# pvjosue/CWFA

Measured on AMD Instinct MI355X. Metric: volumes/sec inverse-pass @512×512×96 fp32; NLL match vs ref (1/2/4/8 GPU), higher is better.
Workload: dtype f32 (storage, accumulation, wavelets, couplings); convolution products on the bf16 matrix cores from an exact three-way bf16 split of both fp32 operands, six products per fp32 product: fp32-equivalent; plain-fp32-MFMA figure: fp32_mfma; 1 GPU; 512x512x96 volume, 4-scale CWFA (CAT blocks, 64 ch) + LRNN inverse, z=0, batch 1/GPU, random-init weights (BASELINE.json configs[2]); precision=split, parallelism=replicated x1 (independent volumes per GPU, no collective)

## Files before the change

### cwfa_amd/_lib.py

```python
import ctypes as C
import os

_HERE = os.path.dirname(os.path.abspath(__file__))
LIB_PATH = os.path.join(_HERE, "libcwfa_hip.so")

CLAMP = {"NONE": 0, "ATAN": 1, "TANH": 2, "SIGMOID": 3}
ACT = {None: 0, "none": 0, "elu": 1, "prelu": 2, "gelu": 3, "relu": 4}
CHAIN_MAX = 8

c_f32p = C.c_void_p
c_i64p = C.c_void_p
c_f64p = C.c_void_p


class AffineStage(C.Structure):
    _fields_ = [("s_raw", c_f32p), ("t", c_f32p), ("s_bs", C.c_int64), ("t_bs", C.c_int64), ("clamp_kind", C.c_int),
                ("clamp", C.c_float), ("pre_scale", C.c_float), ("t_neg_div_sqrt2", C.c_int), ("perm", c_i64p),
                ("perm_axis", C.c_int), ("gin", C.c_int)]


class Chain(C.Structure):
    _fields_ = [("n_stages", C.c_int), ("stage", AffineStage * CHAIN_MAX), ("src_c", C.c_void_p), ("src_h", C.c_void_p)]


# ... 101 lines not shown
    "cwfa_conv2d_wgrad_workspace_bytes": (i64, [i, i, i, i, i, i]),
    "cwfa_conv2d_wgrad_f32": (i, [p, p, p, p, p, i, i, i, i, i, i, i64, i64, f, p]),
    "cwfa_elu_bwd_f32": (i, [p, p, p, p, i, i64, i64, i64, i64, i64, p]),
    "cwfa_conv3d_hidden_fwd_f32": (i, [p, p, p, p, i, i, i, i, i, p]),
    "cwfa_conv3d_hidden_bwd_f32": (i, [p, p, p, p, p, p, i, i, i, i, i, p]),
    "cwfa_conv3d_input_bwd_f32": (i, [p, p, p, i, i, i, i, i, p]),
    "cwfa_conv3d_wgrad_workspace_bytes": (i64, [i, i, i, i]),
    "cwfa_conv3d_wgrad_f32": (i, [p, p, p, p, p, i, i, i, i, i, i, i, f, p]),
    "cwfa_prelu_bwd_f32": (i, [p, p, p, p, p, i, i64, i64, i64, i64, p]),
    "cwfa_plane_affine_f32": (i, [p, p, p, i, p, p, i, i, i64, i64, i64, i64, p]),
    "cwfa_bn_bwd_stats_f32": (i, [p, p, p, p, i, i, i64, i64, i64, p]),
    "cwfa_bn_act_bwd_f32": (i, [p, p, p, i, p, p, p, p, p, i, i, i64, i64, i64, i64, p]),
    "cwfa_maxpool2_bwd_f32": (i, [p, p, p, p, i, i, i, i, p]),
    "cwfa_gelu_f32": (i, [p, p, p, i64, i, p]),
    "cwfa_layernorm_bwd_f32": (i, [p, p, p, p, p, p, p, p, p, i, i64, p]),
    "cwfa_attention_bwd_f32": (i, [p, p, p, p, p, p, p, p, p, i, i, i64, p]),
    "cwfa_split_workspace_bytes": (i64, [i, i, i64]),
    "cwfa_split_input_f32": (i, [p, p, i, i, i64, i64, p, p, i64, p, i64, p]),
    "cwfa_conv_split_packed_bytes": (i64, [i, i, i]),
    "cwfa_conv_split_pack_f32": (i, [p, p, i, i, i, i, p]),
    "cwfa_conv_split_f32": (i, [p, p, p, i, i, i, i, i, i, i64, C.POINTER(ConvOpts), p]),
    "cwfa_conv3x3_split_packed_bytes": (i64, [i, i]),
    "cwfa_conv3x3_split_pack_f32": (i, [p, p, i, i, p]),
    "cwfa_conv3x3_split_f32": (i, [p, p, p, i, i, i, i, i, i64, i64, C.POINTER(ConvOpts), p]),
    "cwfa_conv7x7_split_packed_bytes": (i64, [i, i]),
    "cwfa_conv7x7_split_pack_f32": (i, [p, p, i, i, p]),
    "cwfa_conv7x7_split_f32": (i, [p, p, p, i, i, i, i, i, i64, i64, C.POINTER(ConvOpts), p]),
    "cwfa_couple_rows": (i, [i, p]),
    "cwfa_conv3x3_split_couple_f32": (i, [p, p, p, i, i, i, i, i64, C.POINTER(Couple), p]),
    "cwfa_subnet_layer_split_packed_bytes": (i64, []),
    "cwfa_subnet_layer_split_pack_f32": (i, [p, p, p, p]),
    "cwfa_subnet_layer_split_f32": (i, [p, p, p, p, p, i, i, i, i64, i64, i, p]),
    "cwfa_subnet_layer_split_tape_f32": (i, [p, p, p, p, p, p, i, i, i, i64, i64, i64, p]),
    "cwfa_subnet_layer_first_packed_bytes": (i64, []),
    "cwfa_subnet_layer_first_pack_f32": (i, [p, p, p, i, p, p]),
    "cwfa_subnet_layer_first_f32": (i, [p, p, p, p, p, p, i, i, i, i, i64, i64, i64, i, p]),
    "cwfa_extract_views_f32": (i, [p, p, p, i, i, i, i, i, i, f, f, i64, p]),
    "cwfa_eval_splits": (i64, [i, i64]),
    "cwfa_volume_extrema_f32": (i, [p, p, p, p, i, i64, i64, i64, C.POINTER(EvalAffine), p]),
    "cwfa_volume_metrics_f32": (i, [p, p, p, p, i, i64, i64, i64, C.POINTER(EvalAffine), f, f, f, p]),
    "cwfa_mip3_f32": (i, [p, p, p, p, p, p, i, i, i, i, i64, i64, i, C.POINTER(EvalAffine), C.POINTER(EvalPost), p]),
    "cwfa_projection_compose_f32": (i, [p, p, p, p, p, i, i, i, i, i, i, i, p]),
    "cwfa_roi_means_f32": (i, [p, p, p, i, i, i, i, i, i64, p]),
    "cwfa_select_positive_f32": (i, [p, i, i64, i64, i64, p, p, p, p]),
    "cwfa_prep_volumes_f16": (i, [p, p, p, i, i, i, i, i, i, i, i, i, f, f, i, p]),
    "cwfa_prep_frames_f32": (i, [p, p, i, i, i, i, i, i, i, p]),
    "cwfa_histogram_f32": (i, [p, i64, f, f, p, i, p, i, p]),
    "cwfa_prep_apply_f32": (i, [p, i64, i, f, f, i, p]),
    "cwfa_moments_f64": (i, [p, i64, d, p, p, i, p]),
    "cwfa_stack_mean_std_f32": (i, [p, p, p, i, i64, i64, p]),
    "cwfa_lion_step_f32": (i, [C.POINTER(LionTable), f, f, f, f, p, p, p]),
    "cwfa_wmse_workspace_bytes": (i64, [i64]),
    "cwfa_wmse_loss_f32": (i, [p, p, p, f, f, p, p, p, i64, p]),
    "cwfa_select_nonzero_f32": (i, [p, i, i64, i64, i64, p, p, p, p]),
    "cwfa_deconv_spectrum_mul_c64": (i, [p, p, p, i, i64, i, i, p]),
    "cwfa_deconv_project_f32": (i, [p, p, i, i, i, i, i, i, i, i, i, i, i, p]),
    "cwfa_deconv_ratio_f32": (i, [p, p, p, p, i64, p]),
    "cwfa_deconv_clamp_f32": (i, [p, i64, p, p, f, p]),
    "cwfa_deconv_update_f32": (i, [p, p, i, i, i, i, p]),
}
del i, i64, f, d, p

_lib = None


class CwfaHipError(RuntimeError):
# ... 27 lines not shown
```

### cwfa_amd/build.py

```python
import os
import subprocess
import sys
from concurrent.futures import ThreadPoolExecutor

HERE = os.path.dirname(os.path.abspath(__file__))
CSRC = os.path.join(HERE, "csrc")
INCLUDE = os.path.join(os.path.dirname(HERE), "include")
LIB = os.path.join(HERE, "libcwfa_hip.so")
SOURCES = ["elementwise.hip", "conv2d.hip", "conv_wino.hip", "conv_wino2d.hip", "conv_split_layer.hip", "conv_split3x3.hip", "conv3d.hip", "conv3d_split.hip", "lrnn_ops.hip", "conv_bwd.hip", "eval_ops.hip", "prep_ops.hip", "optim_ops.hip", "loss_ops.hip", "deconv_ops.hip"]
HIPCC = os.environ.get("HIPCC", "/opt/rocm/bin/hipcc")
FLAGS = ["--offload-arch=gfx950", "-O3", "-fPIC", "-std=c++17", "-ffp-contract=off", "-I", INCLUDE, "-I", CSRC,
         "-Wall", "-Wno-unused-function"]


EXTRA = {"conv3d_split.hip": ["-fno-slp-vectorize"]}


def _newer(src, dst):
    return not os.path.exists(dst) or os.path.getmtime(src) > os.path.getmtime(dst)


def build_all(force=False, verbose=False):
    deps = [os.path.join(CSRC, "common.h"), os.path.join(CSRC, "conv_internal.h"), os.path.join(INCLUDE, "cwfa_hip.h"),
            os.path.abspath(__file__)]
    objs, jobs = [], []
    for s in SOURCES:
        src, obj = os.path.join(CSRC, s), os.path.join(CSRC, s.replace(".hip", ".o"))
        objs.append(obj)
        if force or _newer(src, obj) or any(_newer(d, obj) for d in deps):
            jobs.append([HIPCC, *FLAGS, *EXTRA.get(s, []), "-c", src, "-o", obj])

    def run(cmd):
        if verbose:
            print(" ".join(cmd), flush=True)
        r = subprocess.run(cmd, capture_output=True, text=True)
        if r.returncode != 0:
            raise RuntimeError(f"hipcc failed: {' '.join(cmd)}\n{r.stdout}\n{r.stderr}")
        return r.stderr

    with ThreadPoolExecutor(max_workers=4) as ex:
        for warn in ex.map(run, jobs):
            if verbose and warn.strip():
                print(warn, file=sys.stderr)
    if jobs or force or not os.path.exists(LIB) or any(_newer(o, LIB) for o in objs):
        run([HIPCC, "--offload-arch=gfx950", "-shared", "-fPIC", "-o", LIB, *objs])
    return LIB


if __name__ == "__main__":
    print(build_all(force="--force" in sys.argv, verbose=True))
```

### cwfa_amd/networks.py

```python
import glob
import math
import re

import torch
import torch.nn as nn

from . import autograd as AG
from . import ops
from .FrEIA import framework as Ff
from .FrEIA import modules as Fm
from .INN_utils import HaarTransform1D, PermuteDim
from .unet import UNet, _Packed
from .amp import amp_entry

__all__ = ["conditional_wavelet_flow", "wavelet_flow_subnetwork", "wavelet_flow_subnetwork2D",
           "wavelet_flow_subnetwork2D_first", "cond_network", "ResidualBlock", "GlobalAttention", "drop_path", "ConvNeXt",
           "LRNN", "Encoder", "subnet_initialization", "subnet_initialization_small", "zero_initialization",
           "subnet_initialization_positive", "reset_ActNorm", "reset_perm", "serialize_INN_step", "load_INN_steps",
           "HaarTransform1D", "PermuteDim", "UNet"]

networks_n_chans = 64

_CONVS = (nn.Conv2d, nn.Conv3d, nn.Linear)

# ... 81 lines not shown
        if couple is None and AG.tracking(u, conv_in, conv_out, self.block2, self.block4, self.block6):
            a = AG.subnet(self, AG.concat(list(u)) if isinstance(u, (list, tuple)) else u, conv_in, conv_out)
            if out is not None:
                raise NotImplementedError("wavelet_flow_subnetwork: `out=` views are an inference-path feature")
            return a
        P = self._packed.get
        fused = self.n_ch == 64 and all(blk[0].bias is not None and blk[2].bias is not None
                                        for blk in (self.block2, self.block4, self.block6))
        H_, W_ = (u[0] if isinstance(u, (list, tuple)) else u).shape[2:4]
        split_layers = fused and ops._split_bf16 >= 2 and 64 * H_ * W_ * 4 < 2 ** 31
        two = isinstance(u, (list, tuple))
        u1 = None
        if (two and split_layers and ops.FIRST_LAYER_COMPOSED and ops.FIRST_LAYER_FUSED_X and conv_in.kernel_size == (1, 1)
                and conv_in.in_channels <= 31 and sum(t.shape[1] for t in u) == conv_in.in_channels):
            u1 = ops.concat_channels(list(u[:-1]) + [ops.with_ones(u[-1])])
            u, two = u1[:, :-1], False
        if two and not (len(u) == 2 and ops.VIRTUAL_CAT and conv_in.kernel_size == (1, 1) and conv_in.out_channels <= 64):
            u, two = ops.concat_channels(list(u)), False
        pc_in = self._cat_bank(conv_in, u[0].shape[1]) if two else P(conv_in)
        blocked = bool(split_layers and ops.BLOCKED_MAPS and not pc_in.split and pc_in.ks == 1 and pc_in.cout == 64)
        first_form = (split_layers and ops.FIRST_LAYER_COMPOSED and not two and conv_in.kernel_size == (1, 1) and conv_in.in_channels <= 31
                      and not pc_in.split)
        fused_x = first_form and ops.FIRST_LAYER_FUSED_X
        pre = ops.first_map_of(self)
        if fused_x:
            b = None
        elif pre is not None and pre[0] is u and pre[1] is conv_in and blocked:
            b = pre[2]
        elif two:
            b = ops.conv2d(u[0], pc_in, bias=conv_in.bias, out_blocked=blocked, cat=u[1])
        else:
            b = ops.conv2d(u, pc_in, bias=conv_in.bias, out_blocked=blocked)
        pc_out = None if couple is not None else P(conv_out)
        last_reads_blocked = split_layers and ops.BLOCKED_MAPS and (couple is not None or (pc_out.split and pc_out.ks == 3))
        for i, blk in enumerate((self.block2, self.block4, self.block6)):
            if fused:
                if split_layers and i == 0 and first_form:
                    out_blocked = bool(ops.BLOCKED_MAPS)
                    b = ops.subnet_layer_first(u1 if u1 is not None else ops.with_ones(u), b, self._first3(conv_in, blk[0], blk[2]), blk[0].bias, blk[2].bias,
                                               layout=(0 if fused_x else int(blocked)) | (int(out_blocked) << 1))
                    blocked = out_blocked
                    continue
                if split_layers:
                    out_blocked = ops.BLOCKED_MAPS and (i < 2 or last_reads_blocked)
                    b = ops.subnet_layer(b, self._split3(blk[0], blk[2]), blk[0].bias, None, blk[2].bias,
                                         layout=int(blocked) | (int(out_blocked) << 1))
                    blocked = out_blocked
                else:
                    b = ops.subnet_layer(b, P(blk[0]), blk[0].bias, self._panel(blk[2]), blk[2].bias)
                continue
            h = ops.conv2d(b, P(blk[0]), bias=blk[0].bias, act="elu")
            b = ops.conv2d(h, P(blk[2]), bias=blk[2].bias, residual=b, act2="elu")
        if couple is not None:
            return ops.conv3x3_couple(b, self._couple_bank(conv_out), *couple, in_blocked=blocked)
        return ops.conv2d(b, pc_out, bias=conv_out.bias, out=out, in_blocked=blocked)

    def _cat_bank(self, conv, c1):
        w = conv.weight
        pc = self._panels.get(("cat", id(conv), c1))
        if pc is None or pc.version != w._version or pc.src_ptr != w.data_ptr() or pc.epoch != ops.pack_epoch():
            pc = self._panels[("cat", id(conv), c1)] = ops.pack_conv_weight_cat(w, c1)
        return pc

    def _couple_bank(self, conv):
        w, bias = conv.weight, conv.bias
        hit = self._panels.get(("c", id(conv)))
        if hit is not None:
# ... 459 lines not shown
```

### cwfa_amd/ops.py

```python
import ctypes as C

import torch

from . import _lib
from ._lib import AffineStage, Chain, ConvOpts, check

__all__ = ["haar1d", "haar2d", "gather", "affine", "channel_affine", "chain_inv", "chain_inv_var", "chain_inv_roi_cov", "chain_inv_samples", "rand_uniform", "rand_trunc_normal", "chain_nll_map", "nll_compose", "chain_fwd", "pack_conv_weight",
           "conv2d", "conv2d_wgrad", "elu_bwd", "set_precision", "gelu_add", "gelu_bwd", "layernorm_bwd", "attention_bwd", "plane_affine", "bn_bwd_stats", "bn_act_bwd", "maxpool2_bwd", "chain_bwd", "chain_inv_bwd", "prelu_bwd", "conv3d_1k1_backward", "pack_1x1_panel", "pack_split_layer_weight", "subnet_layer", "conv3d_1k1", "channel_stats", "bn_fold", "bn_running_update", "maxpool", "sample_stats", "layernorm_apply",
           "convnext_tail", "conv_writes_sample_stats", "attention_combine", "scale_channels", "axpby", "stage", "lion_step", "global_extrema", "wmse_loss"]


def _stream():
    return C.c_void_p(torch.cuda.current_stream().cuda_stream)


def _p(t):
    return None if t is None else C.c_void_p(t.data_ptr())


def _dev(t, name="tensor"):
    if not torch.is_tensor(t):
        raise TypeError(f"{name}: expected a torch.Tensor, got {type(t)}")
    if not t.is_cuda:
        raise RuntimeError(f"{name}: cwfa_amd runs on MI355X only -- got a {t.device} tensor (no CPU fallback exists)")
# ... 458 lines not shown
    loss = torch.zeros(1, dtype=torch.float64, device=xhat.device)
    if want_low_grad and loss_kind != 0:
        raise ValueError("chain_inv_bwd: dL/dlow is formed from an upstream gradient (loss_kind 0)")
    gz = torch.empty((B, Cc, H, W), dtype=torch.float32, device=xhat.device) if want_latent_grad else None
    glow = torch.empty((B, Cc, H, W), dtype=torch.float32, device=xhat.device) if want_low_grad else None
    check(L.cwfa_chain_inv_bwd_f32(_p(xhat), _p(gt), C.byref(ch), C.byref(gr), B, Cc, H, W, xbs, gbs, float(gscale), int(loss_kind),
                                   int(bool(accumulate)), _p(loss), _p(gz), _p(glow), _stream()), "chain_inv_bwd")
    if want_latent_grad or want_low_grad:
        return loss, gz, glow
    return loss


def chain_bwd(z, stages, grads, final_perm=None, gscale=0.0, ldscale=0.0, gz=None, want_input_grad=False, accumulate=False, gld=None):
    L = _lib.lib()
    z, zbs = planes(z, "z")
    B, Cc, H, W = z.shape
    ch, keep = _chain(stages)
    gr = _chain_grads(grads, (B, Cc, H, W))
    gzbs = 0
    if gz is not None:
        gz, gzbs = planes(gz, "gz")
    gv0 = torch.empty((B, Cc, H, W), dtype=torch.float32, device=z.device) if want_input_grad else None
    if gld is not None:
        gld = _dev(gld, "gld").contiguous()
        if gld.numel() != B:
            raise ValueError("chain_bwd: gld must hold one value per sample")
    check(L.cwfa_chain_bwd_f32(_p(z), _p(gz), C.byref(ch), C.byref(gr), _p(_idx(final_perm)), _p(gv0), B, Cc, H, W, zbs, gzbs,
                               Cc * H * W, float(gscale), float(ldscale), int(bool(accumulate)), _p(gld), _stream()), "chain_bwd")
    return gv0


class PackedConv:
    __slots__ = ("packed", "cout", "cin", "ks", "transposed", "version", "src_ptr", "split", "epoch", "version1", "src_ptr1", "cat_c1",
                 "cat_from", "short")

    def __init__(self, packed, cout, cin, ks, transposed, version, src_ptr, split=False):
        self.packed, self.cout, self.cin, self.ks = packed, cout, cin, ks
        self.transposed, self.version, self.src_ptr = transposed, version, src_ptr
        self.split = split
        self.epoch = _pack_epoch


def pack_conv_weight(w, transposed=False, direct=False):
    L = _lib.lib()
    w = _dev(w, "weight").detach().contiguous()
    if transposed:
        cin, co, kh, kw = w.shape
        if (kh, kw) != (2, 2):
            raise ValueError("only 2x2 stride-2 transposed convolutions are supported")
        cout, ks = 4 * co, 1
    else:
        cout, cin, ks, kw = w.shape
        if ks != kw:
            raise ValueError("square kernels only")
    if direct:
        pass
    elif _split_bf16 and ks == 1 and cout >= 128:
        packed = torch.empty(L.cwfa_conv_split_packed_bytes(cout, cin, ks), dtype=torch.uint8, device=w.device)
        check(L.cwfa_conv_split_pack_f32(_p(w), _p(packed), cout, cin, ks, int(transposed), _stream()), "conv_split_pack")
        return PackedConv(packed, cout, cin, ks, transposed, w._version, w.data_ptr(), split=True)
    narrow_max = 32 if single_product() else SPLIT_3X3_NARROW_MAX
    if not direct and _split_bf16 >= 2 and ks == 3 and cout >= SPLIT_3X3_MIN_COUT and (cout > 32 or (cout <= narrow_max and cin >= 29)):
        packed = torch.empty(L.cwfa_conv3x3_split_packed_bytes(cout, cin), dtype=torch.uint8, device=w.device)
        check(L.cwfa_conv3x3_split_pack_f32(_p(w), _p(packed), cout, cin, _stream()), "conv3x3_split_pack")
        return PackedConv(packed, cout, cin, ks, transposed, w._version, w.data_ptr(), split=True)
    if not direct and SPLIT_7X7 and _split_bf16 >= 2 and ks == 7 and cout <= 64 and cin >= 32:
        packed = torch.empty(L.cwfa_conv7x7_split_packed_bytes(cout, cin), dtype=torch.uint8, device=w.device)
        check(L.cwfa_conv7x7_split_pack_f32(_p(w), _p(packed), cout, cin, _stream()), "conv7x7_split_pack")
        return PackedConv(packed, cout, cin, ks, transposed, w._version, w.data_ptr(), split=True)
    n = L.cwfa_conv2d_packed_floats(cout, cin, ks)
    if n <= 0:
        raise ValueError(f"unsupported filter bank {tuple(w.shape)}")
    packed = torch.empty(n, dtype=torch.float32, device=w.device)
    check(L.cwfa_conv2d_pack_f32(_p(w), _p(packed), cout, cin, ks, int(transposed), _stream()), "conv2d_pack")
    return PackedConv(packed, cout, cin, ks, transposed, w._version, w.data_ptr())


def pack_conv_weight_cat(w, c1):
    w = _dev(w, "weight").detach()
    cout, cin, ks, kw = w.shape
    if ks != 1 or kw != 1 or cout > 64 or not (0 < c1 < cin):
        raise ValueError(f"pack_conv_weight_cat: a 1x1 bank with <= 64 outputs and 0 < c1 < Cin is needed, got {tuple(w.shape)}, c1 = {c1}")
    start = (c1 + 15) // 16 * 16
    wz = torch.zeros((cout, start + cin - c1, 1, 1), dtype=torch.float32, device=w.device)
    wz[:, :c1] = w[:, :c1]
    wz[:, start:] = w[:, c1:]
    pc = pack_conv_weight(wz)
    pc.version, pc.src_ptr = w._version, w.data_ptr()
    pc.cat_c1, pc.cat_from = c1, start
    return pc


def conv_writes_stats(pc, act=None, residual=None, act2=None, out_blocked=False, in_add=False):
    return bool(pc.split and pc.ks == 3 and act in (None, "prelu") and residual is None and act2 is None and not out_blocked
                and not (in_add and act is None))


def conv_writes_sample_stats(pc):
    return bool(pc.split and pc.ks == 7 and pc.cin <= 8)


def conv2d(x, pc, bias=None, act=None, prelu_alpha=None, residual=None, act2=None, in_scale=None, in_shift=None,
           in_add=None, out=None, in_blocked=False, out_blocked=False, cat=None, out_stats=None, out_sample_stats=None):
    L = _lib.lib()
    x, xbs = planes(x, "x")
    B, Cin, H, W = x.shape
    o = ConvOpts()
    keep = [x]
    if cat is not None:
        cat, cbs = planes(cat, "cat")
        c1 = getattr(pc, "cat_c1", None)
        if c1 is None or Cin != c1 or tuple(cat.shape) != (B, pc.cin - pc.cat_from, H, W) or in_scale is not None or in_add is not None:
            raise ValueError("conv2d: `cat` needs a bank from pack_conv_weight_cat for exactly these two inputs, and no load-side prologue")
        o.in_cat, o.in_cat_bs, o.in_cat_from, o.in_cat_c1 = cat.data_ptr(), cbs, pc.cat_from, c1
        keep.append(cat)
        Cin = pc.cin
    if Cin != pc.cin:
        raise ValueError(f"conv2d: input has {Cin} channels, filter bank expects {pc.cin}")
    up = bool(pc.transposed)
    oshape = (B, pc.cout // 4, 2 * H, 2 * W) if up else (B, pc.cout, H, W)
    if out is None:
        out = torch.empty(oshape, dtype=torch.float32, device=x.device)
        ybs = oshape[1] * oshape[2] * oshape[3]
    else:
        if tuple(out.shape) != oshape:
            raise ValueError(f"conv2d: out has shape {tuple(out.shape)}, expected {oshape}")
        out_c, ybs = planes(out, "out")
        if out_c.data_ptr() != out.data_ptr():
            raise ValueError("conv2d: `out` must have contiguous planes")
    if bias is not None:
        o.bias = _dev(bias, "bias").data_ptr()
    o.act, o.act2 = _lib.ACT[act], _lib.ACT[act2]
    if prelu_alpha is not None:
        prelu_alpha = _dev(prelu_alpha, "prelu_alpha")
        o.prelu_alpha = prelu_alpha.data_ptr()
        if prelu_alpha.numel() != 1:
            if prelu_alpha.numel() != pc.cout or not prelu_alpha.is_contiguous() or not (pc.split and pc.ks == 3):
                raise ValueError("conv2d: per-channel PReLU slopes need [Cout] contiguous values and the split-bf16 3x3 kernel")
            o.prelu_per_channel = 1
    elif "prelu" in (act, act2):
        raise ValueError("conv2d: PReLU needs prelu_alpha")
    if residual is not None:
        residual, rbs = planes(residual, "residual")
        if tuple(residual.shape) != oshape:
            raise ValueError(f"conv2d: residual {tuple(residual.shape)} != output {oshape}")
        o.residual, o.res_bs = residual.data_ptr(), rbs
        keep.append(residual)
    if in_scale is not None:
        o.in_scale, o.in_shift = _dev(in_scale).data_ptr(), _dev(in_shift).data_ptr()
        if in_scale.numel() not in (Cin, B * Cin) or in_shift.numel() != in_scale.numel():
            raise ValueError("conv2d: in_scale / in_shift must be [Cin] or [B,Cin]")
        o.in_affine_bs = Cin if (in_scale.numel() == B * Cin and B > 1) else 0
    if in_add is not None:
        in_add, abs_ = planes(in_add, "in_add")
        if tuple(in_add.shape) != tuple(x.shape):
            raise ValueError("conv2d: in_add shape mismatch")
        o.in_add, o.in_add_bs = in_add.data_ptr(), abs_
        keep.append(in_add)
    o.upshuffle2 = int(up)
    if in_blocked:
        if not (pc.split and pc.ks == 3):
            raise ValueError("conv2d: channel-blocked input is read by the split-bf16 3x3 kernel only")
        o.in_blocked8 = 1
    if out_blocked:
        ok3 = (pc.split and pc.ks == 3 and pc.cout % 8 == 0 and residual is None and act2 is None and act in (None, "prelu")
               and not split3x3_narrow(pc.cout) and not (in_add is not None and act is None))
        ok1 = not pc.split and pc.ks == 1 and pc.cout >= 33 and pc.cout % 8 == 0 and not up
        if not (ok3 or ok1):
            raise ValueError("conv2d: channel-blocked output is written by the split-bf16 3x3 kernel (bias / PReLU) and by the "
                             "direct 1x1 kernel with 40..64 output channels only")
        o.out_blocked8 = 1
    if out_stats is not None:
        if not conv_writes_stats(pc, act, residual, act2, out_blocked, in_add is not None):
            raise ValueError("conv2d: out_stats needs the split-bf16 3x3 kernel with an NCHW output and a bias / PReLU epilogue")
        if out_stats.dtype != torch.float64 or out_stats.numel() != 2 * pc.cout or not out_stats.is_cuda:
            raise ValueError("conv2d: out_stats must be a float64 [2*Cout] tensor on the HIP device")
        o.out_stats = out_stats.data_ptr()
    if out_sample_stats is not None:
        if not conv_writes_sample_stats(pc):
            raise ValueError("conv2d: out_sample_stats needs the few-channel split 7x7 kernel (a composed ConvNeXt bank with <= 8 inputs)")
        if out_sample_stats.dtype != torch.float64 or out_sample_stats.numel() != 2 * B or not out_sample_stats.is_cuda:
            raise ValueError("conv2d: out_sample_stats must be a float64 [2*B] tensor on the HIP device")
        o.out_sample_stats = out_sample_stats.data_ptr()
    rec = conv_event_sink
    if rec is not None:
        key = (pc.ks, Cin, pc.cout, H, W, B, "%s|%s|%s|%s|%s" % ("pro" if (in_scale is not None or in_add is not None) else "",
                                                                 act or "", "res" if residual is not None else "", act2 or "",
                                                                 ("up" if up else "") + ("+split" if pc.split else "")),
               in_add is not None)
        if rec.want(key):
            e0, e1 = torch.cuda.Event(enable_timing=True), torch.cuda.Event(enable_timing=True)
            e0.record()
    if pc.split and pc.ks == 7:
        if act or act2 or residual is not None or in_scale is not None or in_add is not None:
            raise ValueError("conv2d: the split-bf16 7x7 kernel has a bias-only epilogue and no load-side prologue")
        check(L.cwfa_conv7x7_split_f32(_p(x), _p(pc.packed), _p(out), B, Cin, H, W, pc.cout, xbs, ybs, C.byref(o), _stream()),
              "conv7x7_split")
    elif pc.split and pc.ks == 3:
        if split3x3_narrow(pc.cout) and (in_scale is not None or in_add is not None):
            if (H * W) % 4 == 0:
                x = plane_affine(x, in_scale, in_shift, add=in_add)
            else:
                if in_scale is not None:
                    if in_scale.numel() == Cin:
                        x = channel_affine(x, in_scale.reshape(-1), in_shift.reshape(-1))
                    else:
                        x = torch.cat([channel_affine(x[i:i + 1], in_scale.reshape(B, Cin)[i].contiguous(), in_shift.reshape(B, Cin)[i].contiguous())
                                       for i in range(B)], 0)
                if in_add is not None:
                    x = axpby(x.contiguous(), 1.0, in_add, 1.0)
            x, xbs = planes(x, "x")
            o.in_scale = o.in_shift = o.in_add = None
        check(L.cwfa_conv3x3_split_f32(_p(x), _p(pc.packed), _p(out), B, Cin, H, W, pc.cout, xbs, ybs, C.byref(o),
                                       _stream()), "conv3x3_split")
    elif pc.split:
        ws = torch.empty(L.cwfa_split_workspace_bytes(B, Cin, H * W), dtype=torch.uint8, device=x.device)
        per_sample = in_scale is not None and in_scale.numel() == B * Cin and B > 1
        check(L.cwfa_split_input_f32(_p(x), _p(ws), B, Cin, H * W, xbs, _p(in_scale), _p(in_shift), Cin if per_sample else 0,
                                     _p(in_add), in_add.stride(0) if in_add is not None else 0, _stream()), "split_input")
        o.in_scale = o.in_shift = o.in_add = None
        check(L.cwfa_conv_split_f32(_p(ws), _p(pc.packed), _p(out), B, Cin, H, W, pc.cout, pc.ks, ybs, C.byref(o), _stream()),
              "conv_split")
    else:
        check(L.cwfa_conv2d_f32(_p(x), _p(pc.packed), _p(out), B, Cin, H, W, pc.cout, pc.ks, xbs, ybs, C.byref(o),
                                _stream()), "conv2d")
    if rec is not None and rec.want(key):
# ... 44 lines not shown
    if logdet is not None:
        cp.logdet = logdet.data_ptr()
    cp.in_blocked8 = int(bool(in_blocked))
    rec = conv_event_sink
    if rec is not None:
        key = (3, Cin, pc.cout, H, W, B, "||||couple+split", False)
        if rec.want(key):
            e0, e1 = torch.cuda.Event(enable_timing=True), torch.cuda.Event(enable_timing=True)
            e0.record()
    check(L.cwfa_conv3x3_split_couple_f32(_p(u), _p(pc.packed), _p(br), B, Cin, H, W, ubs, C.byref(cp), _stream()),
          "conv3x3_split_couple")
    if rec is not None and rec.want(key):
        e1.record()
        rec.add(key, e0, e1)
    return out


BLOCKED_MAPS = True
SPLIT_7X7 = True
VIRTUAL_CAT = True
COUPLE_EPILOGUE = True


def couple_fused():
    return COUPLE_EPILOGUE and _split_bf16 >= 2


def split3x3_narrow(cout):
    return cout <= 48 or 64 < cout <= 96


SPLIT_3X3_MIN_COUT = 1
SPLIT_3X3_NARROW_MAX = 16
conv_event_sink = None


def pack_1x1_panel(w):
    L = _lib.lib()
    w = _dev(w, "weight").detach().contiguous()
    if tuple(w.shape) != (64, 64, 1, 1):
        raise ValueError("pack_1x1_panel: the fused layer kernel is specialised for 64 channels")
    panel = torch.empty(4096, dtype=torch.float32, device=w.device)
    check(L.cwfa_subnet_pack1x1_f32(_p(w), _p(panel), _stream()), "subnet_pack1x1")
    return PackedConv(panel, 64, 64, 1, False, w._version, w.data_ptr())


def pack_split_layer_weight(w3, w1):
    L = _lib.lib()
    w3 = _dev(w3, "weight").detach().contiguous()
    w1 = _dev(w1, "weight").detach().contiguous()
    if tuple(w3.shape) != (64, 64, 3, 3) or tuple(w1.shape) != (64, 64, 1, 1):
        raise ValueError("pack_split_layer_weight: 64x64x3x3 and 64x64x1x1 only")
    packed = torch.empty(L.cwfa_subnet_layer_split_packed_bytes(), dtype=torch.uint8, device=w3.device)
    check(L.cwfa_subnet_layer_split_pack_f32(_p(w3), _p(w1), _p(packed), _stream()), "subnet_layer_split_pack")
    pc = PackedConv(packed, 64, 64, 3, False, w3._version, w3.data_ptr(), split=True)
    pc.version1, pc.src_ptr1 = w1._version, w1.data_ptr()
    return pc


FIRST_LAYER_COMPOSED = True
FIRST_LAYER_FUSED_X = True


def pack_first_layer_weight(w0, b0, w3, w1, short=None):
    L = _lib.lib()
    w0, w3, w1 = _dev(w0, "w0").detach(), _dev(w3, "w3").detach(), _dev(w1, "w1").detach().contiguous()
# ... 1069 lines not shown
```

### include/cwfa_hip.h

```cpp
#ifndef CWFA_HIP_H
#define CWFA_HIP_H

#include <stdint.h>

#ifdef __cplusplus
extern "C" {
#endif

#define CWFA_VERSION 100

enum {
    CWFA_OK = 0,
    CWFA_E_INVAL = -1,
    CWFA_E_SHAPE = -2,
    CWFA_E_ALIGN = -3,
    CWFA_E_HIP = -4
};

enum { CWFA_CLAMP_NONE = 0, CWFA_CLAMP_ATAN = 1, CWFA_CLAMP_TANH = 2, CWFA_CLAMP_SIGMOID = 3 };

enum { CWFA_ACT_NONE = 0, CWFA_ACT_ELU = 1, CWFA_ACT_PRELU = 2, CWFA_ACT_GELU = 3, CWFA_ACT_RELU = 4 };

int cwfa_version(void);
const char* cwfa_last_error(void);
// ... 162 lines not shown
                           int64_t x_bs, int64_t y_bs, const cwfa_conv_opts* opts, void* stream);
int cwfa_conv_split_f32(const void* ws, const void* w_packed, float* y, int B, int Cin, int H, int W, int Cout, int ks, int64_t y_bs,
                           const cwfa_conv_opts* opts, void* stream);
int64_t cwfa_conv7x7_split_packed_bytes(int Cout, int Cin);
int cwfa_conv7x7_split_pack_f32(const float* w, void* packed, int Cout, int Cin, void* stream);
int cwfa_conv7x7_split_f32(const float* x, const void* w_packed, float* y, int B, int Cin, int H, int W, int Cout,
                           int64_t x_bs, int64_t y_bs, const cwfa_conv_opts* opts, void* stream);

typedef struct {
    const float* x;
    float* y;
    int64_t x_bs, y_bs;
    int n;
    int clamp_kind;
    float clamp, pre_scale;
    int rev;
    double* logdet;
    int in_blocked8;
} cwfa_couple;
int cwfa_couple_rows(int n, int* rows);
int cwfa_conv3x3_split_couple_f32(const float* x, const void* w_packed, const float* bias_rows, int B, int Cin, int H, int W,
                                  int64_t x_bs, const cwfa_couple* cp, void* stream);

int64_t cwfa_subnet_layer_split_packed_bytes(void);
int cwfa_subnet_layer_split_pack_f32(const float* w3, const float* w1, void* packed, void* stream);
int cwfa_subnet_layer_split_f32(const float* x, const void* packed, const float* b3, const float* b1, float* y, int B, int H,
                                int W, int64_t x_bs, int64_t y_bs, int layout, void* stream);
int64_t cwfa_subnet_layer_first_packed_bytes(void);
int cwfa_subnet_layer_first_pack_f32(const float* w3c, const float* w1, const float* w0c, int short_form, void* packed, void* stream);
int cwfa_subnet_layer_first_f32(const float* u, const float* x, const void* packed, const float* b3, const float* b1, float* y, int B,
                                int u_ch, int H, int W, int64_t u_bs, int64_t x_bs, int64_t y_bs, int layout, void* stream);
int cwfa_subnet_layer_split_tape_f32(const float* x, const void* packed, const float* b3, const float* b1, float* y, float* hid, int B,
                                     int H, int W, int64_t x_bs, int64_t y_bs, int64_t hid_bs, void* stream);

int cwfa_extract_views_f32(const float* image, const int* coords_yx, float* views, int B, int Hs, int Ws, int nviews, int sh,
                           int sw, float mean, float stdv, int64_t image_bs, void* stream);


typedef struct {
    float* ds[CWFA_CHAIN_MAX];
    float* dt[CWFA_CHAIN_MAX];
    int64_t ds_bs[CWFA_CHAIN_MAX], dt_bs[CWFA_CHAIN_MAX];
} cwfa_chain_grads;

int cwfa_chain_bwd_f32(const float* z, const float* gz, const cwfa_chain* ch, const cwfa_chain_grads* grads,
                       const int64_t* final_perm, float* gv0, int B, int C, int H, int W, int64_t z_bs, int64_t gz_bs,
                       int64_t gv0_bs, float gscale, float ldscale, int accumulate, const float* gld, void* stream);

int cwfa_chain_inv_bwd_f32(const float* xhat, const float* gt, const cwfa_chain* ch, const cwfa_chain_grads* grads, int B, int C,
                           int H, int W, int64_t xhat_bs, int64_t gt_bs, float gscale, int loss_kind, int accumulate,
                           double* loss_sum, float* gz_out, float* glow_out, void* stream);

int cwfa_affine_bwd_f32(const float* x, const float* g, const cwfa_affine_stage* st, int rev, int B, int C, int H, int W,
                        int64_t x_bs, int64_t g_bs, const float* gld, float* gx, float* gs_raw, float* gt_raw, void* stream);

int64_t cwfa_conv2d_wgrad_workspace_bytes(int B, int Cin, int H, int W, int Cout, int ks);
int cwfa_conv2d_wgrad_f32(const float* x, const float* dy, float* dw, float* db, void* workspace, int B, int Cin, int H, int W,
                          int Cout, int ks, int64_t x_bs, int64_t dy_bs, float beta, void* stream);

int cwfa_elu_bwd_f32(const float* g, const float* a, const float* add, float* y, int B, int64_t n, int64_t g_bs, int64_t a_bs,
                     int64_t add_bs, int64_t y_bs, void* stream);

int cwfa_conv3d_hidden_fwd_f32(const float* x, const float* w1, const float* b1, float* q, int B, int D, int H, int W, int K,
                               void* stream);
int cwfa_conv3d_hidden_bwd_f32(const float* dy, const float* w2, const float* q, const float* alpha, float* m, double* dalpha,
                               int B, int D, int H, int W, int K, void* stream);
// ... 98 lines not shown
```

Before: 55.50 volumes/s.

## Add persistent split-bf16 3x3 kernel for narrow subnet output convolutions

Adds a dedicated persistent kernel for the 64-to-at-most-48-channel 3x3 output convolution of the subnetworks. It stages input tiles and weight slices through LDS with double-buffered async loads overlapped with the six-product split MFMA, and walks tiles across CUs (optionally XCD-aware). It can read the channel-blocked input layout, so the preceding layers keep producing blocked maps. The trade-off is a second packed weight copy per eligible conv, and a path that only applies when the epilogue is bias-only.

Result: faster. 56.62 volumes/s (median of 6 runs) (+2.0%).

```diff
diff --git a/cwfa_amd/_lib.py b/cwfa_amd/_lib.py
--- a/cwfa_amd/_lib.py
+++ b/cwfa_amd/_lib.py
@@ -157,6 +157,9 @@
     "cwfa_subnet_layer_split_pack_f32": (i, [p, p, p, p]),
     "cwfa_subnet_layer_split_f32": (i, [p, p, p, p, p, i, i, i, i64, i64, i, p]),
     "cwfa_subnet_layer_split_tape_f32": (i, [p, p, p, p, p, p, i, i, i, i64, i64, i64, p]),
+    "cwfa_conv3x3_out_split_packed_bytes": (i64, [i]),
+    "cwfa_conv3x3_out_split_pack_f32": (i, [p, p, i, p]),
+    "cwfa_conv3x3_out_split_f32": (i, [p, p, p, p, i, i, i, i, i64, i64, i, p]),
     "cwfa_subnet_layer_first_packed_bytes": (i64, []),
     "cwfa_subnet_layer_first_pack_f32": (i, [p, p, p, i, p, p]),
     "cwfa_subnet_layer_first_f32": (i, [p, p, p, p, p, p, i, i, i, i, i64, i64, i64, i, p]),
diff --git a/cwfa_amd/build.py b/cwfa_amd/build.py
--- a/cwfa_amd/build.py
+++ b/cwfa_amd/build.py
@@ -7,7 +7,7 @@
 CSRC = os.path.join(HERE, "csrc")
 INCLUDE = os.path.join(os.path.dirname(HERE), "include")
 LIB = os.path.join(HERE, "libcwfa_hip.so")
-SOURCES = ["elementwise.hip", "conv2d.hip", "conv_wino.hip", "conv_wino2d.hip", "conv_split_layer.hip", "conv_split3x3.hip", "conv3d.hip", "conv3d_split.hip", "lrnn_ops.hip", "conv_bwd.hip", "eval_ops.hip", "prep_ops.hip", "optim_ops.hip", "loss_ops.hip", "deconv_ops.hip"]
+SOURCES = ["elementwise.hip", "conv2d.hip", "conv_wino.hip", "conv_wino2d.hip", "conv_split_layer.hip", "conv_split_out.hip", "conv_split3x3.hip", "conv3d.hip", "conv3d_split.hip", "lrnn_ops.hip", "conv_bwd.hip", "eval_ops.hip", "prep_ops.hip", "optim_ops.hip", "loss_ops.hip", "deconv_ops.hip"]
 HIPCC = os.environ.get("HIPCC", "/opt/rocm/bin/hipcc")
 FLAGS = ["--offload-arch=gfx950", "-O3", "-fPIC", "-std=c++17", "-ffp-contract=off", "-I", INCLUDE, "-I", CSRC,
          "-Wall", "-Wno-unused-function"]
@@ -21,7 +21,7 @@
 
 
 def build_all(force=False, verbose=False):
-    deps = [os.path.join(CSRC, "common.h"), os.path.join(CSRC, "conv_internal.h"), os.path.join(INCLUDE, "cwfa_hip.h"),
+    deps = [os.path.join(CSRC, "common.h"), os.path.join(CSRC, "conv_internal.h"), os.path.join(CSRC, "conv_split_out_geom.h"), os.path.join(INCLUDE, "cwfa_hip.h"),
             os.path.abspath(__file__)]
     objs, jobs = [], []
     for s in SOURCES:
diff --git a/cwfa_amd/csrc/conv_split_out.hip b/cwfa_amd/csrc/conv_split_out.hip
--- /dev/null
+++ b/cwfa_amd/csrc/conv_split_out.hip
@@ -0,0 +1,359 @@
+#include "conv_internal.h"
+#include "conv_split_out_geom.h"
+
+extern int g_cwfa_split_xcd_map;
+
+namespace {
+
+using namespace cwfa_out;
+
+constexpr int XR = TR + 2, XC = TC + 2;
+constexpr int KHB = 9984;
+constexpr int XPB = 2 * KHB;
+constexpr int XB = 3 * XPB;
+constexpr int OFF_W = 2 * XB;
+constexpr int NE = 2 * XR * XC;
+constexpr int lds_bytes(int mt) { return OFF_W + 4 * slice_bytes(mt) + 64 * mt; }
+static_assert(lds_bytes(MAX_MT) <= 160 * 1024, "LDS budget");
+
+struct OParams {
+    const float* x;
+    float* y;
+    const void* wp;
+    const float* bias;
+    int B, H, W, Cout, tiles_x, tiles_y, ntiles;
+    int64_t x_bs, y_bs;
+    int xcd_map;
+};
+
+__host__ __device__ constexpr int unit_off(int u) {
+    const int chunk = u / 9, tap = u % 9;
+    return (chunk & 1) * XB + ((tap / 3) * XC + tap % 3) * 16;
+}
+
+template <bool SIX, bool F16, bool INB, int MT>
+__global__ __launch_bounds__(512, 1) void split_out_kernel(OParams p) {
+    static_assert(MT >= 1 && MT <= MAX_MT, "one to three m-tiles");
+    constexpr int WSL = slice_bytes(MT), OFF_BIAS = OFF_W + 4 * WSL;
+    constexpr int NQ = SIX ? 3 : 1;
+    constexpr int NKB = NQ * MT;
+    constexpr int NST = 16 * MT;
+    extern __shared__ __attribute__((aligned(16))) char lds[];
+    const int tid = threadIdx.x, lane = tid & 63, wave = tid >> 6, c16 = lane & 15, g = lane >> 4;
+    const int HW = p.H * p.W;
+    const int plane = HW * 4;
+    constexpr unsigned OOB = 0x80000000u;
+
+    int epk[3], edst[3];
+    bool fin[3];
+#pragma unroll
+    for (int k = 0; k < 3; ++k) {
+        const int e = tid + k * 512;
+        fin[k] = e < NE;
+        const int c_ = e % XC, r_ = (e / XC) % XR, h_ = (e / (XR * XC)) & 1;
+        epk[k] = c_ | (r_ << 8) | (h_ << 16);
+        edst[k] = h_ * KHB + (r_ * XC + c_) * 16;
+    }
+    const bool stage2 = wave < 4;
+    auto entry_offsets = [&](bool valid, int row0, int col0, unsigned (&fo)[3]) {
+#pragma unroll
+        for (int k = 0; k < 3; ++k) {
+            const int gr = row0 + ((epk[k] >> 8) & 255) - 1, gc = col0 + (epk[k] & 255) - 1, eh = epk[k] >> 16;
+            const bool ok = valid && fin[k] && gr >= 0 && gr < p.H && gc >= 0 && gc < p.W;
+            fo[k] = !ok ? OOB : INB ? (unsigned)((eh * HW + gr * p.W + gc) * 32) : (unsigned)((eh * 8 * HW + gr * p.W + gc) * 4);
+        }
+    };
+    const bool xmap = xcd_walk(p.xcd_map, p.ntiles, (int)gridDim.x);
+    auto coords = [&](int it, int& b, int& row0, int& col0) { tile_coords(it, xmap, p.ntiles, p.tiles_x, p.tiles_y, b, row0, col0); };
+    auto load_entry = [&](f32x4 (&xv)[2], const float* base, unsigned fo, int chunk) {
+        const auto rs = CWFA_RSRC(base, 64 * plane);
+        if constexpr (INB) {
+            xv[0] = __builtin_bit_cast(f32x4, __builtin_amdgcn_raw_buffer_load_b128(rs, fo, chunk * 16 * plane, 0));
+            xv[1] = __builtin_bit_cast(f32x4, __builtin_amdgcn_raw_buffer_load_b128(rs, fo, chunk * 16 * plane + 16, 0));
+            return;
+        }
+#pragma unroll
+        for (int j = 0; j < 8; ++j)
+            xv[j >> 2][j & 3] = __builtin_bit_cast(float, __builtin_amdgcn_raw_buffer_load_b32(rs, fo, (chunk * 16 + j) * plane, 0));
+    };
+    auto store_entry = [&](auto kc, const f32x4 (&xv)[2], int buf) {
+        constexpr int k = decltype(kc)::value;
+        if (k == 2 && !stage2) return;
+        bf16x8 pc[3];
+#pragma unroll
+        for (int j = 0; j < 8; ++j) {
+            __bf16 a1, a2 = (__bf16)0.f, a3 = (__bf16)0.f;
+            cwfa_split3<SIX, F16>(xv[j >> 2][j & 3], a1, a2, a3);
+            pc[0][j] = a1; pc[1][j] = a2; pc[2][j] = a3;
+        }
+        if (fin[k]) {
+            char* dst = lds + buf * XB + edst[k];
+#pragma unroll
+            for (int q = 0; q < NQ; ++q) *reinterpret_cast<bf16x8*>(dst + q * XPB) = pc[q];
+        }
+    };
+
+    const auto rw = CWFA_RSRC(p.wp, NSL * WSL);
+    int tw = 0;
+    auto slot_off = [&](int s) { return (s & 3) * WSL + ((s & 2) ? -tw : tw); };
+    auto dma_w = [&](int s) {
+        const int so = slot_off(s), src = (s % NSL) * WSL;
+        if (wave < NKB)
+            __builtin_amdgcn_raw_ptr_buffer_load_lds(rw, (lds_ptr)(lds + OFF_W + so + wave * 1024), 16, (unsigned)tid * 16u, src, 0, 0);
+        if constexpr (NKB > 8) {
+            if (wave == 0)
+                __builtin_amdgcn_raw_ptr_buffer_load_lds(rw, (lds_ptr)(lds + OFF_W + so + 8192), 16, 8192u + (unsigned)tid * 16u, src, 0, 0);
+        }
+    };
+
+    const int alane = OFF_W + (g * 16 * MT + c16) * 16;
+    const int blane = (g & 1) * KHB + ((2 * wave) * XC + c16) * 16;
+    const bool sel = (g >> 1) != 0;
+    const f32x4* bias4 = reinterpret_cast<const f32x4*>(lds + OFF_BIAS);
+
+    f32x4 acc[MT][4];
+    bf16x8 A[2][3], Bq[4][3];
+    f32x4 xa[3][2], xb[3][2];
+    unsigned fo_c[3], fo_n[3];
+
+    auto read_a = [&](int set, int s, int mt) {
+        const int ab = alane + slot_off(s);
+#pragma unroll
+        for (int q = 0; q < NQ; ++q) A[set][q] = *reinterpret_cast<const bf16x8*>(lds + ab + (q * 64 * MT + mt * 16) * 16);
+    };
+    auto read_b = [&](int nt, int bbase) {
+#pragma unroll
+        for (int q = 0; q < NQ; ++q)
+            Bq[nt][q] = *reinterpret_cast<const bf16x8*>(lds + bbase + q * XPB + ((nt >> 1) * XC + 16 * (nt & 1)) * 16);
+    };
+    auto mfma6 = [&](f32x4& c, const bf16x8 (&a)[3], const bf16x8 (&b)[3]) {
+        if constexpr (SIX) {
+            CWFA_MFMA(a[2], b[0], c);
+            CWFA_MFMA(a[1], b[1], c);
+            CWFA_MFMA(a[0], b[2], c);
+            CWFA_MFMA(a[1], b[0], c);
+            CWFA_MFMA(a[0], b[1], c);
+        }
+        CWFA_MFMA_OP(F16, a[0], b[0], c);
+    };
+    auto bbase_of = [&](int offA, int offB) { return blane + (sel ? offB : offA); };
+
+    if (tid < 16 * MT) reinterpret_cast<float*>(lds + OFF_BIAS)[tid] = (p.bias != nullptr && tid < p.Cout) ? p.bias[tid] : 0.f;
+    int tile = blockIdx.x;
+    int tb, row0, col0;
+    coords(tile, tb, row0, col0);
+    const float* xs_cur = p.x + (int64_t)tb * p.x_bs;
+    entry_offsets(true, row0, col0, fo_c);
+    cwfa_static_for<3>([&](auto kc) { load_entry(xa[decltype(kc)::value], xs_cur, fo_c[decltype(kc)::value], 0); });
+    cwfa_static_for<3>([&](auto kc) { load_entry(xb[decltype(kc)::value], xs_cur, fo_c[decltype(kc)::value], 1); });
+    dma_w(0);
+    dma_w(1);
+    dma_w(2);
+    dma_w(3);
+    cwfa_static_for<3>([&](auto kc) { store_entry(kc, xa[decltype(kc)::value], 0); });
+    asm volatile("s_waitcnt vmcnt(0)\n\ts_waitcnt lgkmcnt(0)" ::: "memory");
+    __builtin_amdgcn_s_barrier();
+    read_a(0, 0, 0);
+    {
+        const int bb = bbase_of(unit_off(0), unit_off(1));
+#pragma unroll
+        for (int nt = 0; nt < 4; ++nt) read_b(nt, bb);
+    }
+
+    for (; tile < p.ntiles; tile += gridDim.x) {
+        const int ntile = tile + gridDim.x;
+        const bool has_next = ntile < p.ntiles;
+        int nb, nrow0, ncol0;
+        coords(has_next ? ntile : tile, nb, nrow0, ncol0);
+        const float* xs_next = p.x + (int64_t)nb * p.x_bs;
+        entry_offsets(has_next, nrow0, ncol0, fo_n);
+
+#pragma unroll
+        for (int mt = 0; mt < MT; ++mt) {
+            const f32x4 bv = bias4[mt * 4 + g];
+#pragma unroll
+            for (int nt = 0; nt < 4; ++nt) acc[mt][nt] = bv;
+        }
+
+        cwfa_static_for<NSL>([&](auto sc) {
+            constexpr int S = decltype(sc)::value, P = S % 9, PER = S / 9;
+            constexpr bool LASTP = PER == 1;
+            constexpr auto loads_in = [](int s) { return ((s % 9 >= 2 && s % 9 <= 4) || s % 9 >= 6) ? (INB ? 2 : 8) : 0; };
+            constexpr int NL = loads_in(S), NLP = loads_in((S + NSL - 1) % NSL);
+            auto issue_memory = [&]() {
+                if constexpr (S != 0) dma_w(S + 3);
+                if constexpr (P >= 2 && P <= 4) {
+                    constexpr int k = P - 2;
+                    if constexpr (!LASTP) load_entry(xa[k], xs_cur, fo_c[k], 2 * PER + 2);
+                    else load_entry(xa[k], xs_next, fo_n[k], 0);
+                }
+                if constexpr (P >= 6) {
+                    constexpr int k = P - 6;
+                    if constexpr (!LASTP) load_entry(xb[k], xs_cur, fo_c[k], 2 * PER + 3);
+                    else load_entry(xb[k], xs_next, fo_n[k], 1);
+                }
+            };
+            constexpr int NS = (S + 1) % NSL;
+            const int bbn = bbase_of(unit_off(2 * NS), unit_off(2 * NS + 1));
+            CWFA_FENCE();
+#pragma unroll
+            for (int mt = 0; mt < MT; ++mt) {
+                const int set = (S * MT + mt) & 1;
+                if (mt < MT - 1) read_a(set ^ 1, S, mt + 1);
+                else read_a(set ^ 1, S + 1, 0);
+                CWFA_FENCE();
+#pragma unroll
+                for (int np = 0; np < 4; np += 2) {
+                    mfma6(acc[mt][np], A[set], Bq[np]);
+                    mfma6(acc[mt][np + 1], A[set], Bq[np + 1]);
+                    CWFA_FENCE();
+                    if (mt == MT - 1) {
+                        read_b(np, bbn);
+                        read_b(np + 1, bbn);
+                        CWFA_FENCE();
+                    }
+                }
+                if (mt == 0) {
+                    issue_memory();
+                    CWFA_FENCE();
+                    if constexpr (P <= 2) store_entry(cwfa_ic<P>{}, xb[P], 1);
+                    if constexpr (P >= 5 && P <= 7) store_entry(cwfa_ic<P - 5>{}, xa[P - 5], 0);
+                    CWFA_FENCE();
+                }
+            }
+            asm volatile("s_waitcnt vmcnt(%0)" ::"n"(S == 0 ? NLP + NST : S == 1 ? NST : NLP + NL) : "memory");
+            asm volatile("s_waitcnt lgkmcnt(0)" ::: "memory");
+            __builtin_amdgcn_s_barrier();
+        });
+
+        dma_w(NSL + 3);
+        {
+            const auto ry = CWFA_RSRC(p.y + (int64_t)tb * p.y_bs, p.Cout * plane);
+#pragma unroll
+            for (int nt = 0; nt < 4; ++nt) {
+                const int row = row0 + 2 * wave + (nt >> 1), col = col0 + 16 * (nt & 1) + c16;
+                const bool ok = col < p.W && row < p.H;
+                const unsigned oo = (unsigned)(row * p.W + col) * 4u + (unsigned)g * 4u * (unsigned)plane;
+#pragma unroll
+                for (int mt = 0; mt < MT; ++mt)
+#pragma unroll
+                    for (int r = 0; r < 4; ++r) {
+                        const float v = acc[mt][nt][r];
+                        __builtin_amdgcn_raw_buffer_store_b32(__builtin_bit_cast(unsigned, v), ry,
+                                                              (ok && mt * 16 + 4 * g + r < p.Cout) ? oo : OOB, (mt * 16 + r) * plane, 0);
+                    }
+            }
+        }
+        tb = nb; row0 = nrow0; col0 = ncol0;
+        xs_cur = xs_next;
+        tw = 2 * WSL - tw;
+#pragma unroll
+        for (int k = 0; k < 3; ++k) fo_c[k] = fo_n[k];
+    }
+    asm volatile("s_waitcnt vmcnt(0)" ::: "memory");
+}
+
+template <bool F16>
+__global__ __launch_bounds__(256) void split_out_pack_kernel(const float* __restrict__ w, uint4* __restrict__ out, int Cout, int mt) {
+    const int i = blockIdx.x * blockDim.x + threadIdx.x;
+    const int rows = 16 * mt;
+    if (i >= NSL * 4 * rows) return;
+    const int co = i % rows, g = (i / rows) % 4, sl = i / (4 * rows);
+    unsigned short pc[3][8];
+#pragma unroll
+    for (int j = 0; j < 8; ++j) {
+        const float v = co < Cout ? w[pack_src(sl, g, j, co)] : 0.f;
+        __bf16 a1, a2, a3;
+        if constexpr (F16) {
+            cwfa_split3<false, true>(v, a1, a2, a3);
+            a2 = a3 = __builtin_bit_cast(__bf16, (unsigned short)0);
+        } else {
+            cwfa_split3<true>(v, a1, a2, a3);
+        }
+        pc[0][j] = __builtin_bit_cast(unsigned short, a1);
+        pc[1][j] = __builtin_bit_cast(unsigned short, a2);
+        pc[2][j] = __builtin_bit_cast(unsigned short, a3);
+    }
+#pragma unroll
+    for (int q = 0; q < 3; ++q) {
+        uint4 u;
+        u.x = pc[q][0] | ((unsigned)pc[q][1] << 16);
+        u.y = pc[q][2] | ((unsigned)pc[q][3] << 16);
+        u.z = pc[q][4] | ((unsigned)pc[q][5] << 16);
+        u.w = pc[q][6] | ((unsigned)pc[q][7] << 16);
+        out[pack_dst(sl, q, g, co, mt)] = u;
+    }
+}
+
+int g_out_cus = 0;
+
+template <bool SIX, bool F16, bool INB, int MT>
+int out_launch(const OParams& p, int grid, hipStream_t st) {
+    constexpr auto kern = &split_out_kernel<SIX, F16, INB, MT>;
+    const int rc = cwfa_max_lds<kern>(lds_bytes(MT), "cwfa_conv3x3_out_split_f32");
+    if (rc) return rc;
+    hipLaunchKernelGGL(kern, dim3(grid), dim3(512), lds_bytes(MT), st, p);
+    CWFA_LAUNCH_CHECK("cwfa_conv3x3_out_split_f32");
+    return CWFA_OK;
+}
+
+}
+
+extern "C" int64_t cwfa_conv3x3_out_split_packed_bytes(int Cout) {
+    if (Cout < 1 || Cout > MAX_COUT) return -1;
+    return packed_bytes(Cout);
+}
+
+extern "C" int cwfa_conv3x3_out_split_pack_f32(const float* w, void* packed, int Cout, void* stream) {
+    CWFA_REQUIRE(w && packed, CWFA_E_INVAL, "cwfa_conv3x3_out_split_pack_f32: null pointer");
+    CWFA_REQUIRE(Cout >= 1 && Cout <= MAX_COUT, CWFA_E_SHAPE, "cwfa_conv3x3_out_split_pack_f32: 1 <= Cout <= 48 (got %d)", Cout);
+    CWFA_REQUIRE(cwfa_aligned16(packed), CWFA_E_ALIGN, "cwfa_conv3x3_out_split_pack_f32: packed image must be 16-byte aligned");
+    const int mt = mt_of(Cout);
+    const dim3 grid((unsigned)((NSL * 4 * 16 * mt + 255) / 256));
+    uint4* out = reinterpret_cast<uint4*>(packed);
+    cwfa_with_operand([&](auto, auto f16) -> int {
+        hipLaunchKernelGGL(split_out_pack_kernel<f16>, grid, dim3(256), 0, (hipStream_t)stream, w, out, Cout, mt);
+        return CWFA_OK;
+    });
+    CWFA_LAUNCH_CHECK("cwfa_conv3x3_out_split_pack_f32");
+    return CWFA_OK;
+}
+
+extern "C" int cwfa_conv3x3_out_split_f32(const float* x, const void* packed, const float* bias, float* y, int B, int H, int W, int Cout,
+                                          int64_t x_bs, int64_t y_bs, int in_blocked, void* stream) {
+    CWFA_REQUIRE(Cout >= 1 && Cout <= MAX_COUT, CWFA_E_SHAPE, "cwfa_conv3x3_out_split_f32: 1 <= Cout <= 48 (got %d)", Cout);
+    CWFA_REQUIRE(B >= 0 && H >= 0 && W >= 0, CWFA_E_INVAL, "cwfa_conv3x3_out_split_f32: bad size");
+    if (B == 0 || H == 0 || W == 0) return CWFA_OK;
+    CWFA_REQUIRE(x && packed && y, CWFA_E_INVAL, "cwfa_conv3x3_out_split_f32: null pointer");
+    CWFA_REQUIRE((const void*)x != (const void*)y, CWFA_E_INVAL, "cwfa_conv3x3_out_split_f32: in-place not supported (3x3 halo)");
+    CWFA_REQUIRE(cwfa_aligned16(packed), CWFA_E_ALIGN, "cwfa_conv3x3_out_split_f32: packed image must be 16-byte aligned");
+    CWFA_REQUIRE(!in_blocked || cwfa_aligned16(x), CWFA_E_ALIGN, "cwfa_conv3x3_out_split_f32: blocked input must be 16-byte aligned");
+    CWFA_REQUIRE(!in_blocked || (x_bs & 3) == 0, CWFA_E_ALIGN, "cwfa_conv3x3_out_split_f32: blocked input batch stride must be a multiple of 4");
+    CWFA_REQUIRE((int64_t)CIN * H * W * 4 < (1ll << 31), CWFA_E_SHAPE, "cwfa_conv3x3_out_split_f32: image too large for 32-bit offsets");
+    const Walk wk = walk_of(B, H, W);
+    CWFA_REQUIRE(wk.ntiles < (1ll << 31), CWFA_E_SHAPE, "cwfa_conv3x3_out_split_f32: too many tiles");
+    OParams p{};
+    p.x = x; p.y = y; p.wp = packed; p.bias = bias;
+    p.B = B; p.H = H; p.W = W; p.Cout = Cout; p.x_bs = x_bs; p.y_bs = y_bs;
+    p.tiles_x = wk.tiles_x; p.tiles_y = wk.tiles_y; p.ntiles = (int)wk.ntiles;
+    p.xcd_map = g_cwfa_split_xcd_map;
+    if (g_out_cus == 0) {
+        int dev = 0, n = 0;
+        if (hipGetDevice(&dev) != hipSuccess || hipDeviceGetAttribute(&n, hipDeviceAttributeMultiprocessorCount, dev) != hipSuccess || n <= 0) {
+            cwfa_set_error("cwfa_conv3x3_out_split_f32: cannot query the CU count");
+            return CWFA_E_HIP;
+        }
+        g_out_cus = n;
+    }
+    const int grid = grid_of(wk.ntiles, g_out_cus);
+    const hipStream_t st = (hipStream_t)stream;
+    const int mt = mt_of(Cout);
+    return cwfa_with_operand([&](auto six, auto f16) -> int {
+        auto go = [&](auto inb) -> int {
+            if (mt == 1) return out_launch<six, f16, inb, 1>(p, grid, st);
+            if (mt == 2) return out_launch<six, f16, inb, 2>(p, grid, st);
+            return out_launch<six, f16, inb, 3>(p, grid, st);
+        };
+        return in_blocked ? go(std::true_type{}) : go(std::false_type{});
+    });
+}
diff --git a/cwfa_amd/csrc/conv_split_out_geom.h b/cwfa_amd/csrc/conv_split_out_geom.h
--- /dev/null
+++ b/cwfa_amd/csrc/conv_split_out_geom.h
@@ -0,0 +1,46 @@
+#pragma once
+#include <cstdint>
+
+#if defined(__HIPCC__) || defined(__CUDACC__)
+#define CWFA_GEOM_HD __host__ __device__
+#else
+#define CWFA_GEOM_HD
+#endif
+
+namespace cwfa_out {
+
+constexpr int TR = 16, TC = 32;
+constexpr int CIN = 64, NSL = 18;
+constexpr int MAX_COUT = 48, MAX_MT = 3;
+
+CWFA_GEOM_HD constexpr int mt_of(int cout) { return (cout + 15) / 16; }
+CWFA_GEOM_HD constexpr int slice_bytes(int mt) { return 3 * 4 * 16 * mt * 16; }
+CWFA_GEOM_HD constexpr int64_t packed_bytes(int cout) { return (int64_t)NSL * slice_bytes(mt_of(cout)); }
+
+CWFA_GEOM_HD constexpr int pack_dst(int sl, int q, int g, int co, int mt) { return (sl * 3 + q) * (64 * mt) + g * 16 * mt + co; }
+CWFA_GEOM_HD constexpr int64_t pack_src(int sl, int g, int j, int co) {
+    const int u = 2 * sl + (g >> 1), c = u / 9, t = u % 9;
+    return ((int64_t)co * CIN + c * 16 + (g & 1) * 8 + j) * 9 + t;
+}
+
+struct Walk {
+    int tiles_x, tiles_y;
+    int64_t ntiles;
+};
+CWFA_GEOM_HD constexpr Walk walk_of(int B, int H, int W) {
+    const int tx = (W + TC - 1) / TC, ty = (H + TR - 1) / TR;
+    return Walk{tx, ty, (int64_t)tx * ty * B};
+}
+CWFA_GEOM_HD constexpr int grid_of(int64_t ntiles, int cus) { return (int)(ntiles < cus ? ntiles : cus); }
+CWFA_GEOM_HD constexpr bool xcd_walk(int xcd_map, int ntiles, int grid) { return xcd_map && (ntiles & 7) == 0 && (grid & 7) == 0; }
+CWFA_GEOM_HD constexpr void tile_coords(int it, bool xmap, int ntiles, int tiles_x, int tiles_y, int& b, int& row0, int& col0) {
+    const int tile = xmap ? (it & 7) * (ntiles >> 3) + (it >> 3) : it;
+    const int per = tiles_x * tiles_y;
+    b = tile / per;
+    const int rem = tile - b * per;
+    const int ty = rem / tiles_x;
+    row0 = ty * TR;
+    col0 = (rem - ty * tiles_x) * TC;
+}
+
+}
diff --git a/cwfa_amd/networks.py b/cwfa_amd/networks.py
--- a/cwfa_amd/networks.py
+++ b/cwfa_amd/networks.py
@@ -137,7 +137,7 @@
         else:
             b = ops.conv2d(u, pc_in, bias=conv_in.bias, out_blocked=blocked)
         pc_out = None if couple is not None else P(conv_out)
-        last_reads_blocked = split_layers and ops.BLOCKED_MAPS and (couple is not None or (pc_out.split and pc_out.ks == 3))
+        last_reads_blocked = split_layers and ops.BLOCKED_MAPS and (couple is not None or (pc_out.split and pc_out.ks == 3) or ops.out_walk_selected(pc_out, H_, W_))
         for i, blk in enumerate((self.block2, self.block4, self.block6)):
             if fused:
                 if split_layers and i == 0 and first_form:
diff --git a/cwfa_amd/ops.py b/cwfa_amd/ops.py
--- a/cwfa_amd/ops.py
+++ b/cwfa_amd/ops.py
@@ -514,16 +514,27 @@
 
 class PackedConv:
     __slots__ = ("packed", "cout", "cin", "ks", "transposed", "version", "src_ptr", "split", "epoch", "version1", "src_ptr1", "cat_c1",
-                 "cat_from", "short")
+                 "cat_from", "short", "walk")
 
     def __init__(self, packed, cout, cin, ks, transposed, version, src_ptr, split=False):
         self.packed, self.cout, self.cin, self.ks = packed, cout, cin, ks
         self.transposed, self.version, self.src_ptr = transposed, version, src_ptr
         self.split = split
         self.epoch = _pack_epoch
+        self.walk = None
 
 
 def pack_conv_weight(w, transposed=False, direct=False):
+    pc = _pack_conv_weight(w, transposed, direct)
+    if not direct and out_walk_bank(pc.cout, pc.cin, pc.ks, transposed):
+        L = _lib.lib()
+        wc = _dev(w, "weight").detach().contiguous()
+        pc.walk = torch.empty(L.cwfa_conv3x3_out_split_packed_bytes(pc.cout), dtype=torch.uint8, device=wc.device)
+        check(L.cwfa_conv3x3_out_split_pack_f32(_p(wc), _p(pc.walk), pc.cout, _stream()), "conv3x3_out_split_pack")
+    return pc
+
+
+def _pack_conv_weight(w, transposed, direct):
     L = _lib.lib()
     w = _dev(w, "weight").detach().contiguous()
     if transposed:
@@ -589,6 +600,8 @@
     B, Cin, H, W = x.shape
     o = ConvOpts()
     keep = [x]
+    walk = out_walk_selected(pc, H, W, act=act, prelu_alpha=prelu_alpha, residual=residual, act2=act2, in_scale=in_scale, in_add=in_add,
+                             out_blocked=out_blocked, cat=cat, out_stats=out_stats, out_sample_stats=out_sample_stats)
     if cat is not None:
         cat, cbs = planes(cat, "cat")
         c1 = getattr(pc, "cat_c1", None)
@@ -641,8 +654,8 @@
         keep.append(in_add)
     o.upshuffle2 = int(up)
     if in_blocked:
-        if not (pc.split and pc.ks == 3):
-            raise ValueError("conv2d: channel-blocked input is read by the split-bf16 3x3 kernel only")
+        if not (walk or (pc.split and pc.ks == 3)):
+            raise ValueError("conv2d: channel-blocked input is read by the split-bf16 3x3 kernels only")
         o.in_blocked8 = 1
     if out_blocked:
         ok3 = (pc.split and pc.ks == 3 and pc.cout % 8 == 0 and residual is None and act2 is None and act in (None, "prelu")
@@ -673,7 +686,10 @@
         if rec.want(key):
             e0, e1 = torch.cuda.Event(enable_timing=True), torch.cuda.Event(enable_timing=True)
             e0.record()
-    if pc.split and pc.ks == 7:
+    if walk:
+        check(L.cwfa_conv3x3_out_split_f32(_p(x), _p(pc.walk), _p(bias), _p(out), B, H, W, pc.cout, xbs, ybs, int(bool(in_blocked)),
+                                           _stream()), "conv3x3_out_split")
+    elif pc.split and pc.ks == 7:
         if act or act2 or residual is not None or in_scale is not None or in_add is not None:
             raise ValueError("conv2d: the split-bf16 7x7 kernel has a bias-only epilogue and no load-side prologue")
         check(L.cwfa_conv7x7_split_f32(_p(x), _p(pc.packed), _p(out), B, Cin, H, W, pc.cout, xbs, ybs, C.byref(o), _stream()),
@@ -784,6 +800,22 @@
 
 SPLIT_3X3_MIN_COUT = 1
 SPLIT_3X3_NARROW_MAX = 16
+OUT_WALK = True
+OUT_WALK_MT = (1, 2, 3)
+
+
+def out_walk_bank(cout, cin, ks, transposed=False):
+    return bool(OUT_WALK and _split_bf16 >= 2 and ks == 3 and not transposed and cin == 64 and 1 <= cout <= 48
+                and (cout + 15) // 16 in OUT_WALK_MT)
+
+
+def out_walk_selected(pc, H, W, act=None, prelu_alpha=None, residual=None, act2=None, in_scale=None, in_add=None, out_blocked=False,
+                      cat=None, out_stats=None, out_sample_stats=None):
+    return bool(OUT_WALK and getattr(pc, "walk", None) is not None and act is None and prelu_alpha is None
+                and residual is None and act2 is None and in_scale is None and in_add is None and not out_blocked and cat is None
+                and out_stats is None and out_sample_stats is None and 64 * H * W * 4 < 2 ** 31)
+
+
 conv_event_sink = None
 
 
diff --git a/include/cwfa_hip.h b/include/cwfa_hip.h
--- a/include/cwfa_hip.h
+++ b/include/cwfa_hip.h
@@ -218,6 +218,10 @@
                                 int u_ch, int H, int W, int64_t u_bs, int64_t x_bs, int64_t y_bs, int layout, void* stream);
 int cwfa_subnet_layer_split_tape_f32(const float* x, const void* packed, const float* b3, const float* b1, float* y, float* hid, int B,
                                      int H, int W, int64_t x_bs, int64_t y_bs, int64_t hid_bs, void* stream);
+int64_t cwfa_conv3x3_out_split_packed_bytes(int Cout);
+int cwfa_conv3x3_out_split_pack_f32(const float* w, void* packed, int Cout, void* stream);
+int cwfa_conv3x3_out_split_f32(const float* x, const void* packed, const float* bias, float* y, int B, int H, int W, int Cout,
+                               int64_t x_bs, int64_t y_bs, int in_blocked, void* stream);
 
 int cwfa_extract_views_f32(const float* image, const int* coords_yx, float* views, int B, int Hs, int Ws, int nviews, int sh,
                            int sw, float mean, float stdv, int64_t image_bs, void* stream);
```
